# zwizwa/synth_tools

Hardware: NVIDIA B200
Metric: voice-samples/sec (higher is better)
Workload: dtype u32

## Files before the change

### synth_tools_b200/csrc/common.cuh

```cuda
#pragma once
#include <cuda_runtime.h>
#include <stdint.h>
#include <string>
#include <vector>
#include "../../include/cproc_cuda.h"

#define CPROC_N_SM 148

struct cproc_cuda_ctx {
    int device = 0;
    cudaStream_t stream = nullptr;
    cudaStream_t copy_stream = nullptr;
    cudaStream_t aux_stream = nullptr;
    cudaEvent_t aux_ev[17] = {};
    bool own_stream = false;
    cudaEvent_t ev0 = nullptr, ev1 = nullptr;
    std::string err;
    uint64_t launches = 0;
    int pdm_block = 64;
    int pdm_tpb = 2;
    int pdm_stage = 1;
    int pdm_ws = 1;
    int pdm_tlog = 7;
    int pdm_v1_chains = 2;
    int pdm_planar_bulk = 2;
    int pdm_ctas_per_sm = 4;
    int pdm_slice_batches = 64;
    uint32_t *d_work = nullptr;
    uint32_t *d_sm_rank = nullptr;
    uint32_t *d_jump[5] = {nullptr, nullptr, nullptr, nullptr, nullptr};
    uint32_t *d_jump16 = nullptr;
    int pdm_persist = 1;
    int pdm_warps_per_smsp = 1;
    int n_sm = CPROC_N_SM;
    int voice_fpt = 0;
    int grain_block = 128;
    int grain_blocks_per_sm = 2;
    int grain_bulk = 5;
    int grain_vec4 = 1;
    int grain_mix2 = 2;
    int planar_bulk = 2;
    int graph_vec4 = 1;
    int graph_jit = 1;
    int xvoice_vpt = 0;
    int xvoice_mix2_per_sm = 0;
    int xvoice_mix2_blocks = 0;
    int xvoice_mix2 = 1;
    int xvoice_groups = 0;
    int xvoice_chunk = 0;
    uint64_t opt_epoch = 0;
    int run_graph = 2;
    int xvoice_closed = 1;
};

struct cproc_graph_jit {
    int state = 0;
    std::vector<char> cubin;
    cudaLibrary_t lib = nullptr;
    cudaKernel_t k_il = nullptr, k_il4 = nullptr, k_pl = nullptr, k_ps = nullptr, k_pt = nullptr;
    uint32_t pl_smem = 0, pl_block = 0, pt_smem = 0;
};

struct cproc_cuda_bus;
struct cproc_cuda_batch {
    cproc_cuda_ctx *ctx = nullptr;
    cproc_cuda_bus *bus = nullptr; uint32_t bus_mode = 0;
    cproc_cuda_config cfg{};
    std::vector<cproc_cuda_node> nodes;
    std::vector<uint32_t> node_off;
    std::vector<uint32_t> outs;
    uint64_t n = 0;
    uint64_t npad = 0;
    uint64_t n_banks = 0;
    uint64_t n_bus = 0;
    uint32_t state_words = 0, param_words = 0;
    uint32_t *d_state = nullptr;
    uint32_t *d_param = nullptr;
    uint32_t *d_prng = nullptr;
    uint32_t *d_prng2 = nullptr;
    uint32_t *d_prng_g = nullptr;
    cproc_cuda_node *d_nodes = nullptr;
    uint32_t count = 0;
    void *d_in = nullptr, *d_in2 = nullptr, *d_ctl = nullptr, *d_out = nullptr, *d_mix = nullptr;
    size_t cap_in = 0, cap_in2 = 0, cap_ctl = 0, cap_out = 0, cap_mix = 0;
    void *d_out2 = nullptr; size_t cap_out2 = 0;
    uint32_t *d_aux = nullptr; bool aux_dirty = true; uint32_t aux_weird = 0;
    void *d_scratch = nullptr; size_t cap_scratch = 0;
    uint32_t *d_acc = nullptr; size_t cap_acc = 0;
    unsigned long long *d_flags = nullptr;
    uint64_t n_flags = 0;
    unsigned long long epoch = 0;
    cproc_graph_jit jit[2];
    std::vector<uint32_t> ev_in, ev_chg, ev_out;
    std::string jit_log;
    struct run_graph {
        uint64_t F = 0; uint32_t layout = 0; size_t sz[5] = {0, 0, 0, 0, 0};
        uint64_t opt_epoch = 0;
        int seen = 0;
        cudaGraphExec_t exec = nullptr; uint32_t kernels = 0;
        uint8_t *h = nullptr; size_t cap = 0;
    } rg;
    uint32_t *st_h = nullptr; bool ride_state = false;
};

int cproc_set_err(cproc_cuda_ctx *ctx, int code, const char *fmt, ...);
int cproc_check(cproc_cuda_ctx *ctx, cudaError_t e, const char *what);

#define CK(ctx, call) do { int _rc = cproc_check((ctx), (call), #call); if (_rc) return _rc; } while (0)
#define CK_LAUNCH(ctx, name) do { (ctx)->launches++; int _rc = cproc_check((ctx), cudaGetLastError(), name); if (_rc) return _rc; } while (0)

struct cproc_kind_meta {
    const char *name;
    uint32_t n_state; const char *state[5]; uint32_t state_f;
    uint32_t n_param; const char *param[3]; uint32_t param_f;
    uint32_t n_input; const char *input[2]; uint32_t input_f;
    uint32_t n_config; const char *config[1];
};
static const cproc_kind_meta k_cproc_kinds[CPROC_CUDA_NODE_KINDS] = {
    {"acc",      1, {"out"}, 0,                                    0, {nullptr}, 0,                               1, {"in"}, 0,           0, {nullptr}},
    {"edge",     2, {"out", "last"}, 0,                            0, {nullptr}, 0,                               1, {"in"}, 0,           0, {nullptr}},
    {"glide",    5, {"out", "vel0", "pos1", "vel1", "count"}, 0,   0, {nullptr}, 0,                               1, {"in"}, 0,           1, {"div_log"}},
    {"pdm",      5, {"out", "s1", "s2", "s3", "s4"}, 0,            0, {nullptr}, 0,                               2, {"in", "dither"}, 0, 1, {"order_shift"}},
    {"phasor_f", 2, {"out", "phase"}, 1,                           1, {"inc"}, 0,                                 1, {"mod"}, 0,          0, {nullptr}},
    {"svf",      2, {"out", "bp"}, 3,                              2, {"f", "q"}, 3,                              1, {"in"}, 1,           0, {nullptr}},
    {"env",      3, {"out", "env", "t"}, 3,                        3, {"attack", "release", "gate_frames"}, 3,    1, {"in"}, 1,           0, {nullptr}},
    {"onepole",  1, {"out"}, 1,                                    1, {"a"}, 1,                                   1, {"in"}, 1,           0, {nullptr}},
    {"gain",     1, {"out"}, 1,                                    1, {"g"}, 1,                                   1, {"in"}, 1,           0, {nullptr}},
    {"asfloat",  1, {"out"}, 1,                                    0, {nullptr}, 0,                               1, {"in"}, 0,           0, {nullptr}},
    {"glide_f",  3, {"out", "step", "count"}, 3,                   0, {nullptr}, 0,                               1, {"in"}, 1,           1, {"div_log"}},
    {"mul",      1, {"out"}, 1,                                    0, {nullptr}, 0,                               2, {"in", "gain"}, 3,   0, {nullptr}},
};
static inline bool cproc_kind_out_float(uint32_t type) { const uint32_t k = CPROC_CUDA_NODE_KIND(type); return k < CPROC_CUDA_NODE_KINDS && (k_cproc_kinds[k].state_f & 1u); }
static inline uint32_t cproc_node_words(uint32_t type) {
    const uint32_t kind = CPROC_CUDA_NODE_KIND(type);
    if (kind == CPROC_CUDA_NODE_PDM) return 1u + (CPROC_CUDA_NODE_ARG(type) & 7u);
    return kind < CPROC_CUDA_NODE_KINDS ? k_cproc_kinds[kind].n_state : 1u;
}
static inline uint32_t cproc_node_param_words(uint32_t type) {
    const uint32_t kind = CPROC_CUDA_NODE_KIND(type);
    return kind < CPROC_CUDA_NODE_KINDS ? k_cproc_kinds[kind].n_param : 0u;
}
static inline const char *cproc_node_check(const cproc_cuda_node *nodes, uint32_t k, uint32_t n_inputs) {
    const cproc_cuda_node &nd = nodes[k];
    const uint32_t kind = CPROC_CUDA_NODE_KIND(nd.type), arg = CPROC_CUDA_NODE_ARG(nd.type);
    if (kind >= CPROC_CUDA_NODE_KINDS || (nd.type >> 16)) return "unknown node type";
    if ((kind == CPROC_CUDA_NODE_GLIDE || kind == CPROC_CUDA_NODE_GLIDE_F) && (arg < 1 || arg > 24)) return "glide needs a control divider log2 of 1..24";
    if (kind == CPROC_CUDA_NODE_PDM && ((arg & 7u) < 1 || (arg & 7u) > 4)) return "pdm order must be 1..4";
    if (kind != CPROC_CUDA_NODE_GLIDE && kind != CPROC_CUDA_NODE_GLIDE_F && kind != CPROC_CUDA_NODE_PDM && arg) return "this processor takes no config word";
    const cproc_kind_meta &m = k_cproc_kinds[kind];
    for (uint32_t j = 0; j < m.n_input; ++j) {
        const int32_t src = j ? nd.src2 : nd.src;
        if (src == CPROC_CUDA_SRC_ZERO) { if (kind <= CPROC_CUDA_NODE_PDM) return "input not connected"; continue; }
        if (src >= (int32_t)k) return j ? "second input reads a node that is not bound yet (ANF)" : "reads a node that is not bound yet (ANF)";
        if (src < 0 && (uint32_t)(-(src + 1)) >= n_inputs) return j ? "second input reads an input stream that does not exist" : "reads an input stream that does not exist";
        if (src >= 0 && cproc_kind_out_float(nodes[src].type) && !((m.input_f >> j) & 1u)) return "a float output feeds an integer input (undefined in C for negative values)";
    }
    return nullptr;
}
static inline uint64_t ceil_div_u64(uint64_t a, uint64_t b) { return (a + b - 1) / b; }

struct cproc_io_sizes { size_t in, in2, ctl, out, mix; };
int cproc_io_bytes(const cproc_cuda_batch *b, uint64_t F, const cproc_cuda_io *io, cproc_io_sizes *s);

int launch_graph(cproc_cuda_batch *b, uint64_t F, const cproc_cuda_io *io);
int launch_graph_scan(cproc_cuda_batch *b, uint64_t F, const cproc_cuda_io *io);
int cproc_graph_jit_get(cproc_cuda_batch *b, bool has_changed, cproc_graph_jit **out);
int launch_pdm(cproc_cuda_batch *b, uint64_t F, const cproc_cuda_io *io);
int launch_pdm_v1(cproc_cuda_batch *b, uint64_t F, const cproc_cuda_io *io);
int launch_pdm_v2(cproc_cuda_batch *b, uint64_t F, const cproc_cuda_io *io);
int launch_pwm(cproc_cuda_batch *b, uint64_t F, const cproc_cuda_io *io);
int launch_voice_bank(cproc_cuda_batch *b, uint64_t F, const cproc_cuda_io *io);
int launch_square_grain(cproc_cuda_batch *b, uint64_t F, const cproc_cuda_io *io);
int launch_square_grain_mix(cproc_cuda_batch *b, uint64_t F, const cproc_cuda_io *io);
int launch_xvoice(cproc_cuda_batch *b, uint64_t F, const cproc_cuda_io *io);
int launch_onepole(cproc_cuda_batch *b, uint64_t F, const cproc_cuda_io *io);
int launch_word_clock(cproc_cuda_batch *b, uint64_t F, const cproc_cuda_io *io);

__global__ void k_imix_to_float(const int32_t *imix, float *mix, uint64_t count, float scale);
__global__ void k_voice_finish(const int32_t *isum, float *vec, uint64_t count, uint32_t mode);

__device__ __forceinline__ uint32_t xorshift32_step(uint32_t x) {
    x ^= x << 13;
    x ^= x >> 17;
    x ^= x << 5;
    return x;
}

__device__ __forceinline__ void st_v4_stream(void *p, uint4 v) {
    asm volatile("st.global.cs.v4.u32 [%0], {%1, %2, %3, %4};" ::"l"(p), "r"(v.x), "r"(v.y), "r"(v.z), "r"(v.w) : "memory");
}
__device__ __forceinline__ uint4 ld_v4_stream(const void *p) {
    uint4 v;
    asm volatile("ld.global.cs.v4.u32 {%0, %1, %2, %3}, [%4];" : "=r"(v.x), "=r"(v.y), "=r"(v.z), "=r"(v.w) : "l"(p));
    return v;
}
```

### synth_tools_b200/csrc/k_pdm_v2.cu

```cuda
#include "common.cuh"
#include "pdm_common.cuh"
#include "planar_bulk.cuh"

struct PdmV2Params {
    uint32_t *st;
    uint64_t npad, n, n_banks;
    uint32_t bank_size;
    const uint32_t *prng;
    uint32_t *prng_out;
    const uint32_t *dither_ext;
    const uint32_t *setpoints;
    uint8_t *out;
    uint64_t F;
    uint32_t count0, ctl_div_log, sh, dmask, layout;
    uint32_t m1;
};

template <int K, int B>
struct V2Regs {
    uint32_t sp[B], p0[B], v0[B], p1[B], v1[B], s[B][K];
    __device__ __forceinline__ void load(const uint32_t *st, uint64_t npad, uint64_t c0) {
#pragma unroll
        for (int j = 0; j < B; ++j) {
            const uint32_t *x = st + c0 + j;
            sp[j] = __ldcg(x); p0[j] = __ldcg(x + npad); v0[j] = __ldcg(x + 2 * npad);
            p1[j] = __ldcg(x + 3 * npad); v1[j] = __ldcg(x + 4 * npad);
#pragma unroll
            for (int k = 0; k < K; ++k) s[j][k] = __ldcg(x + (5 + k) * npad);
        }
    }
    __device__ __forceinline__ void zero() {
#pragma unroll
        for (int j = 0; j < B; ++j) {
            sp[j] = p0[j] = v0[j] = p1[j] = v1[j] = 0;
#pragma unroll
            for (int k = 0; k < K; ++k) s[j][k] = 0;
        }
    }
    __device__ __forceinline__ void store(uint32_t *st, uint64_t npad, uint64_t c0) const {
#pragma unroll
        for (int j = 0; j < B; ++j) {
            uint32_t *x = st + c0 + j;
            __stcg(x, sp[j]); __stcg(x + npad, p0[j]); __stcg(x + 2 * npad, v0[j]);
            __stcg(x + 3 * npad, p1[j]); __stcg(x + 4 * npad, v1[j]);
#pragma unroll
            for (int k = 0; k < K; ++k) __stcg(x + (5 + k) * npad, s[j][k]);
        }
    }
    __device__ __forceinline__ void boundary(const uint32_t *row, uint64_t c0, uint64_t n, uint32_t L) {
#pragma unroll
        for (int j = 0; j < B; ++j) {
            if (row && c0 + j < n) sp[j] = __ldg(row + c0 + j);
            p0[j] = p1[j]; v0[j] = v1[j];
            p1[j] += v1[j] << L;
            v1[j] = (uint32_t)((int32_t)(sp[j] - p1[j]) >> L);
        }
    }
    template <bool FASTQ, bool DEXT>
    __device__ __forceinline__ void group(uint32_t &rng, const uint32_t *dext16, uint32_t sh, uint32_t dmask, uint32_t m1, uint32_t (&w)[B][4]) {
        uint32_t dbuf[16];
        if (DEXT) {
#pragma unroll
            for (int i = 0; i < 4; ++i) {
                uint4 v = *reinterpret_cast<const uint4 *>(dext16 + i * 4);
                dbuf[4 * i] = v.x; dbuf[4 * i + 1] = v.y; dbuf[4 * i + 2] = v.z; dbuf[4 * i + 3] = v.w;
            }
        }
        uint32_t a[B][4];
#pragma unroll
        for (int i = 0; i < 16; ++i) {
            uint32_t d;
            if (DEXT) d = dbuf[i] & dmask;
            else { rng = xorshift32_step(rng); asm("and.b32 %0, %1, %2;" : "=r"(d) : "r"(rng), "r"(dmask)); }
#pragma unroll
            for (int j = 0; j < B; ++j) {
                p0[j] += v0[j];
                if (FASTQ) a[j][i & 3] = pdm_step_q24<K>(s[j], p0[j], d, m1);
                else a[j][i & 3] = pdm_step<K>(s[j], p0[j], sh, d);
                if ((i & 3) == 3)
                    w[j][i >> 2] = FASTQ ? pack_top_bytes(a[j][0], a[j][1], a[j][2], a[j][3])
                                         : pack_low_bytes(a[j][0], a[j][1], a[j][2], a[j][3]);
            }
        }
    }
};

__device__ __forceinline__ uint64_t v2_rows_before(uint32_t count0, uint32_t div, uint64_t t0) {
    const uint64_t first = count0 == 0 ? 0 : div - count0;
    return t0 > first ? 1 + (t0 - first - 1) / div : 0;
}

template <int K, int B, bool TPB, bool FASTQ, bool DEXT>
__global__ void __launch_bounds__(128) k_pdm_v2_simple(const PdmV2Params p) {
    const uint64_t tid = (uint64_t)blockIdx.x * blockDim.x + threadIdx.x;
    if (tid >= (TPB ? p.n_banks : p.n_banks * p.bank_size)) return;
    const uint64_t c0 = tid * B;
    const uint64_t bank = TPB ? tid : tid / p.bank_size;
    const bool rng_owner = TPB ? true : (tid % p.bank_size == 0);
    V2Regs<K, B> r;
    r.load(p.st, p.npad, c0);
    uint32_t rng = __ldg(p.prng + bank);
    const uint32_t L = p.ctl_div_log, div_mask = (1u << L) - 1u;
    uint32_t cnt = p.count0;
    uint64_t row = 0;
    const uint32_t *dext = DEXT ? p.dither_ext + bank * p.F : nullptr;
    const bool tiled = p.layout == CPROC_CUDA_TILED;
    for (uint64_t g = 0; g < (p.F >> 4); ++g) {
        if (cnt == 0) {
            r.boundary(p.setpoints ? p.setpoints + row * p.n : nullptr, c0, p.n, L);
            ++row;
        }
        uint32_t w[B][4];
        r.template group<FASTQ, DEXT>(rng, DEXT ? dext + (g << 4) : nullptr, p.sh, p.dmask, p.m1, w);
#pragma unroll
        for (int j = 0; j < B; ++j) {
            if (c0 + j < p.n) {
                uint8_t *dst = tiled ? p.out + ((g * p.n + c0 + j) << 4) : p.out + (c0 + j) * p.F + (g << 4);
                st_v4_stream(dst, make_uint4(w[j][0], w[j][1], w[j][2], w[j][3]));
            }
        }
        cnt = (cnt + 16) & div_mask;
    }
    r.store(p.st, p.npad, c0);
    if (rng_owner && !DEXT) p.prng_out[bank] = rng;
}

template <int K>
__global__ void k_pdm_v2_any(const PdmV2Params p) {
    const uint64_t c = (uint64_t)blockIdx.x * blockDim.x + threadIdx.x;
    if (c >= p.n_banks * p.bank_size) return;
    const uint64_t bank = c / p.bank_size;
    uint32_t *x = p.st + c;
    uint32_t sp = x[0], p0 = x[p.npad], v0 = x[2 * p.npad], p1 = x[3 * p.npad], v1 = x[4 * p.npad], s[K];
#pragma unroll
    for (int k = 0; k < K; ++k) s[k] = x[(5 + k) * p.npad];
    uint32_t rng = __ldg(p.prng + bank);
    const uint32_t L = p.ctl_div_log, div_mask = (1u << L) - 1u;
    uint32_t cnt = p.count0;
    uint64_t row = 0;
    const uint32_t *dext = p.dither_ext ? p.dither_ext + bank * p.F : nullptr;
    for (uint64_t t = 0; t < p.F; ++t) {
        uint32_t d = dext ? dext[t] : (rng = xorshift32_step(rng));
        d &= p.dmask;
        if (cnt == 0) {
            if (p.setpoints && c < p.n) sp = p.setpoints[row * p.n + c];
            p0 = p1; v0 = v1;
            p1 += v1 << L;
            v1 = (uint32_t)((int32_t)(sp - p1) >> L);
            ++row;
        }
        p0 += v0;
        uint32_t q = pdm_step<K>(s, p0, p.sh, d);
        if (c < p.n) {
            uint64_t idx = p.layout == CPROC_CUDA_TILED ? (((t >> 4) * p.n + c) << 4) + (t & 15)
                         : p.layout == CPROC_CUDA_INTERLEAVED ? t * p.n + c
                         : c * p.F + t;
            p.out[idx] = (uint8_t)q;
        }
        cnt = (cnt + 1) & div_mask;
    }
    x[0] = sp; x[p.npad] = p0; x[2 * p.npad] = v0; x[3 * p.npad] = p1; x[4 * p.npad] = v1;
#pragma unroll
    for (int k = 0; k < K; ++k) x[(5 + k) * p.npad] = s[k];
    if (!dext && c % p.bank_size == 0) p.prng_out[bank] = rng;
}

#define WS4_BAR_FULL 1
#define WS4_BAR_EMPTY 3
template <int ID, int N> __device__ __forceinline__ void bar_sync_i() { asm volatile("bar.sync %0, %1;" ::"n"(ID), "n"(N) : "memory"); }
template <int ID, int N> __device__ __forceinline__ void bar_arrive_i() { asm volatile("bar.arrive %0, %1;" ::"n"(ID), "n"(N) : "memory"); }
template <int BASE, int N> __device__ __forceinline__ void bar_sync_slot(uint32_t s) { if (s) bar_sync_i<BASE + 1, N>(); else bar_sync_i<BASE, N>(); }
template <int BASE, int N> __device__ __forceinline__ void bar_arrive_slot(uint32_t s) { if (s) bar_arrive_i<BASE + 1, N>(); else bar_arrive_i<BASE, N>(); }

struct PdmV2Work {
    uint32_t *counter;
    unsigned long long *flags;
    unsigned long long epoch;
    uint32_t groups, slices, bps;
    uint32_t *prng_g;
    uint32_t *sm_rank;
    const uint32_t *jump;
};

template <int K>
__device__ __forceinline__ uint32_t ws4_tick(uint32_t &p0, uint32_t v0, uint32_t (&s)[K], uint32_t d, uint32_t m1) {
    p0 += v0;
    if constexpr (K == 2) {
        const uint32_t x = s[0] + p0;
        const uint32_t a = lop3_and_or(s[1], d);
        s[0] = imad(a, m1, x);
        s[1] = s[1] + s[0] - a;
        return a;
    } else {
        return pdm_step_q24<K>(s, p0, d, m1);
    }
}

template <int NT, int TLOG>
__device__ __noinline__ uint32_t ws4_producer_arith(uint4 *dbuf, const uint32_t (*jt)[256], uint32_t x0, uint32_t dmask, uint64_t batches, uint32_t lane) {
    constexpr int QW = (1 << TLOG) / 4, QC = QW / 2;
    uint32_t xa = x0, s = 0;
    for (uint64_t bt = 0; bt < batches; ++bt) {
        uint32_t xb = jump_apply(jt, xa);
        if (bt >= 2) bar_sync_slot<WS4_BAR_EMPTY, NT>(s);
        uint4 *slot = dbuf + s * (QW * 32) + lane;
#pragma unroll 4
        for (int q = 0; q < QC; ++q) {
            uint4 va, vb;
            xa = xorshift32_step(xa); va.x = xa & dmask;
            xb = xorshift32_step(xb); vb.x = xb & dmask;
            xa = xorshift32_step(xa); va.y = xa & dmask;
            xb = xorshift32_step(xb); vb.y = xb & dmask;
            xa = xorshift32_step(xa); va.z = xa & dmask;
            xb = xorshift32_step(xb); vb.z = xb & dmask;
            xa = xorshift32_step(xa); va.w = xa & dmask;
            xb = xorshift32_step(xb); vb.w = xb & dmask;
            slot[q * 32] = va;
            slot[(QC + q) * 32] = vb;
        }
        xa = xb;
        __threadfence_block();
        bar_arrive_slot<WS4_BAR_FULL, NT>(s);
        s ^= 1u;
    }
    return xa;
}

constexpr size_t ws4_smem_bytes(int CW, int TLOG, int PL) {
    return (size_t)(PL == 2 ? CW * 2 * 4096 : PL == 1 ? CW * 4096 : 0) + 2 * ((1u << TLOG) / 4) * 32 * 16 + 4096 + 1024;
}

template <int K, int CW, int TLOG, int PL>
__global__ void __launch_bounds__(32 * (CW + 1)) k_pdm_v2_ws4(const PdmV2Params p, const PdmV2Work wk, const __grid_constant__ CUtensorMap tm_out) {
    constexpr int T = 1 << TLOG, NT = 32 * (CW + 1);
    constexpr int QW = T / 4;
    extern __shared__ __align__(1024) uint8_t ws4_smem[];
    uint8_t *base = ws4_smem + ((1024u - ((uint32_t)__cvta_generic_to_shared(ws4_smem) & 1023u)) & 1023u);
    uint8_t *pbox = base;
    uint4 *dbuf = reinterpret_cast<uint4 *>(base + (PL == 2 ? CW * 2 * 4096 : PL == 1 ? CW * 4096 : 0));
    uint32_t *tab = reinterpret_cast<uint32_t *>(dbuf + 2 * QW * 32);
    for (uint32_t i = threadIdx.x; i < 1024; i += NT) tab[i] = __ldg(wk.jump + i);
    __shared__ uint32_t rank_s, smsp_s[CW + 1], item_s;
    const uint32_t warp = threadIdx.x >> 5, lane = threadIdx.x & 31;
    if (threadIdx.x == 0) {
        uint32_t smid;
        asm volatile("mov.u32 %0, %%smid;" : "=r"(smid));
        rank_s = atomicAdd(wk.sm_rank + smid, 1u);
    }
    if (lane == 0) {
        uint32_t wid;
        asm volatile("mov.u32 %0, %%warpid;" : "=r"(wid));
        smsp_s[warp] = wid & 3u;
    }
    __syncthreads();
    uint32_t prod_warp = 0;
#pragma unroll
    for (int w = CW; w >= 0; --w) if (smsp_s[w] == (rank_s & 3u)) prod_warp = w;
    const uint32_t cw = warp - (warp > prod_warp ? 1u : 0u);
    const uint32_t cl = cw * 32 + lane;
    const uint32_t L = p.ctl_div_log, period = 1u << (L - TLOG);
    const uint32_t m1 = p.m1, bs = p.bank_size;
    const uint64_t batches_total = p.F >> TLOG;
    const uint64_t n_ch = p.n_banks * bs;
    const uint32_t total = wk.groups * wk.slices;
    for (;;) {
        if (threadIdx.x == 0) {
            const uint32_t idx = atomicAdd(wk.counter, 1u);
            item_s = idx;
            if (idx < total) {
                const uint32_t g = idx % wk.groups, sl = idx / wk.groups;
                const unsigned long long want = (wk.epoch << 32) | sl;
                if (sl) while (ld_acquire_u64(wk.flags + g) != want) __nanosleep(64);
            }
        }
        __syncthreads();
        const uint32_t idx = item_s;
        if (idx >= total) break;
        const uint32_t g = idx % wk.groups, sl = idx / wk.groups;
        const uint64_t bt0 = (uint64_t)sl * wk.bps;
        const uint64_t nb = batches_total - bt0 < wk.bps ? batches_total - bt0 : wk.bps;
        const uint64_t c_lo = (uint64_t)g * (32 * CW);
        const uint64_t bank_lo = c_lo / bs;
        if (warp == prod_warp) {
            const uint64_t bank = bank_lo + lane;
            const bool have = bank < p.n_banks;
            uint32_t x = 1u;
            if (have) x = sl ? __ldcg(wk.prng_g + (uint64_t)g * 32 + lane) : __ldg(p.prng + bank);
            x = ws4_producer_arith<NT, TLOG>(dbuf, reinterpret_cast<const uint32_t (*)[256]>(tab), x, p.dmask, nb, lane);
            if (have) {
                if (sl + 1 < wk.slices) __stcg(wk.prng_g + (uint64_t)g * 32 + lane, x);
                else if (bank * bs >= c_lo && bank * bs < c_lo + 32 * CW) p.prng_out[bank] = x;
            }
        } else {
            const uint64_t c = c_lo + cl;
            const bool live = c < n_ch;
            const uint32_t bl = live ? (uint32_t)(c / bs - bank_lo) : 0u;
            V2Regs<K, 1> r;
            if (live) r.load(p.st, p.npad, c); else r.zero();
            const uint32_t cb = (uint32_t)(((p.count0 >> TLOG) + bt0) & (period - 1));
            uint32_t until = cb == 0 ? 0 : period - cb;
            const uint32_t *sp_row = p.setpoints ? p.setpoints + v2_rows_before(p.count0, 1u << L, bt0 << TLOG) * p.n : nullptr;
            const bool store = c < p.n;
            uint8_t *dst = p.layout == CPROC_CUDA_TILED ? p.out + (((bt0 << (TLOG - 4)) * p.n + c) << 4) : p.out + c * p.F + (bt0 << TLOG);
            const uint64_t dstep = p.layout == CPROC_CUDA_TILED ? p.n << 4 : 16;
            const uint32_t pbox_s = PL == 2 ? (uint32_t)__cvta_generic_to_shared(pbox + cw * 8192) : PL == 1 ? (uint32_t)__cvta_generic_to_shared(pbox) : 0u;
            const uint4 *dlane = dbuf + bl;
            uint32_t s = 0;
            for (uint64_t bt = 0; bt < nb; ++bt) {
                if (until == 0) {
                    r.boundary(sp_row, c, p.n, L);
                    if (sp_row) sp_row += p.n;
                    until = period;
                }
                --until;
                bar_sync_slot<WS4_BAR_FULL, NT>(s);
                const uint4 *dslot = dlane + s * (QW * 32);
#pragma unroll
                for (int g16 = 0; g16 < T / 16; ++g16) {
                    uint32_t w[4];
#pragma unroll
                    for (int i4 = 0; i4 < 4; ++i4) {
                        const uint4 dv = dslot[(g16 * 4 + i4) * 32];
                        const uint32_t d[4] = {dv.x, dv.y, dv.z, dv.w};
                        uint32_t a[4];
#pragma unroll
                        for (int i = 0; i < 4; ++i) a[i] = ws4_tick<K>(r.p0[0], r.v0[0], r.s[0], d[i], m1);
                        if constexpr (PL == 1) {
                            const uint32_t row = (((uint32_t)bt << TLOG) + g16 * 16 + i4 * 4) & 127u;
#pragma unroll
                            for (int i = 0; i < 4; ++i)
                                asm volatile("st.shared.u8 [%0], %1;" ::"r"(pbox_s + (row + i) * (32u * CW) + cl), "r"(a[i] >> 24) : "memory");
                        } else w[i4] = pack_top_bytes(a[0], a[1], a[2], a[3]);
                    }
                    if constexpr (PL == 1) {
                        const uint32_t tk = ((uint32_t)bt << TLOG) + g16 * 16;
                        if ((tk & 127u) == 112u) {
                            bar_sync_i<5, 32 * CW>();
                            const uint64_t tick0 = (bt0 << TLOG) + tk - 112;
#pragma unroll
                            for (int i = 0; i < 8; ++i) {
                                const uint32_t piece = i * (32u * CW) + cl, row = piece / (2u * CW), col = piece % (2u * CW);
                                if (c_lo + col * 16 < p.n) {
                                    uint4 v;
                                    asm volatile("ld.shared.v4.u32 {%0, %1, %2, %3}, [%4];" : "=r"(v.x), "=r"(v.y), "=r"(v.z), "=r"(v.w) : "r"(pbox_s + piece * 16u));
                                    st_v4_stream(p.out + (tick0 + row) * p.n + c_lo + col * 16, v);
                                }
                            }
                        }
                    } else if constexpr (PL == 2) {
                        const uint32_t tk = ((uint32_t)bt << TLOG) + g16 * 16;
                        const uint32_t box = (tk >> 7) & 1u, ch = (tk >> 4) & 7u;
                        if (ch == 0 && tk >= 256) {
                            if (lane == 0) asm volatile("cp.async.bulk.wait_group.read 1;" ::: "memory");
                            __syncwarp();
                        }
                        asm volatile("st.shared.v4.u32 [%0], {%1, %2, %3, %4};" ::"r"(pbox_s + box * 4096u + lane * 128u + ((ch ^ (lane & 7u)) << 4)),
                                     "r"(w[0]), "r"(w[1]), "r"(w[2]), "r"(w[3]) : "memory");
                        if (ch == 7) {
                            asm volatile("fence.proxy.async.shared::cta;" ::: "memory");
                            __syncwarp();
                            if (lane == 0) {
                                asm volatile("cp.async.bulk.tensor.2d.global.shared::cta.tile.bulk_group [%0, {%1, %2}], [%3];"
                                             ::"l"(reinterpret_cast<uint64_t>(&tm_out)), "r"((int32_t)((bt0 << TLOG) + tk - 112)), "r"((int32_t)(c_lo + cw * 32)),
                                               "r"(pbox_s + box * 4096u) : "memory");
                                asm volatile("cp.async.bulk.commit_group;" ::: "memory");
                            }
                        }
                    } else {
                        if (store) st_v4_stream(dst, make_uint4(w[0], w[1], w[2], w[3]));
                        dst += dstep;
                    }
                }
                if (bt + 2 < nb) bar_arrive_slot<WS4_BAR_EMPTY, NT>(s);
                s ^= 1u;
            }
            if constexpr (PL == 2) {
                if (lane == 0) asm volatile("cp.async.bulk.wait_group.read 0;" ::: "memory");
                __syncwarp();
            }
            if (live) r.store(p.st, p.npad, c);
        }
        __syncthreads();
        if (threadIdx.x == 0) {
            __threadfence();
            st_release_u64(wk.flags + g, (wk.epoch << 32) | (sl + 1));
        }
    }
    if (threadIdx.x == 0) {
        const uint32_t left = atomicAdd(wk.counter + 1, 1u);
        if (left == gridDim.x - 1) { wk.counter[0] = 0; wk.counter[1] = 0; __threadfence(); }
    }
}


static int ws4_jump(cproc_cuda_ctx *ctx, int tlog, const uint32_t **out) {
    uint32_t *&d = ctx->d_jump[tlog - 6];
    if (!d) {
        std::vector<uint32_t> h(1024);
        jump_table_fill(h.data(), 1u << (tlog - 1));
        CK(ctx, cudaMalloc(&d, h.size() * 4));
        CK(ctx, cudaMemcpyAsync(d, h.data(), h.size() * 4, cudaMemcpyHostToDevice, ctx->stream));
        CK(ctx, cudaStreamSynchronize(ctx->stream));
    }
    *out = d;
    return 0;
}

template <int K, int CW, int TLOG, int PL>
static int ws4_go(cproc_cuda_ctx *ctx, const PdmV2Params &p, PdmV2Work &wk, const CUtensorMap &tm, uint64_t slice_ticks) {
    auto kern = k_pdm_v2_ws4<K, CW, TLOG, PL>;
    constexpr size_t smem = ws4_smem_bytes(CW, TLOG, PL);
    static int occ = 0;
    if (!occ) {
        CK(ctx, cudaFuncSetAttribute(kern, cudaFuncAttributeMaxDynamicSharedMemorySize, (int)smem));
        CK(ctx, cudaOccupancyMaxActiveBlocksPerMultiprocessor(&occ, kern, 32 * (CW + 1), smem));
        if (occ < 1) { occ = 0; return cproc_set_err(ctx, CPROC_CUDA_ECUDA, "pdm_v2: kernel does not fit an SM (%zu bytes of shared memory)", smem); }
    }
    const uint64_t batches = p.F >> TLOG;
    uint64_t bps = slice_ticks >> TLOG;
    if (PL != 0 && TLOG < 7) bps &= ~(uint64_t)((128 >> TLOG) - 1);
    if (bps < 1) bps = PL != 0 && TLOG < 7 ? (128 >> TLOG) : 1;
    wk.bps = (uint32_t)bps;
    wk.slices = (uint32_t)ceil_div_u64(batches, bps);
    if ((uint64_t)wk.groups * wk.slices >= 0xFFFFFFFFull) return cproc_set_err(ctx, CPROC_CUDA_EINVAL, "pdm_v2: too many work items; render fewer ticks per call");
    int want_per_sm = ctx->pdm_ctas_per_sm;
    if (CW == 1 && want_per_sm < 6) want_per_sm = 6;
    const int per_sm = want_per_sm < occ ? want_per_sm : occ;
    uint64_t grid = (uint64_t)ctx->n_sm * per_sm;
    if (grid > wk.groups) grid = wk.groups;
    kern<<<(unsigned)grid, 32 * (CW + 1), smem, ctx->stream>>>(p, wk, tm);
    return 0;
}

template <int K, int CW>
static int ws4_dispatch(cproc_cuda_ctx *ctx, const PdmV2Params &p, PdmV2Work &wk, const CUtensorMap &tm, int tlog, int pl, uint64_t slice_ticks) {
    if (pl == 1) return ws4_go<K, CW, 7, 1>(ctx, p, wk, tm, slice_ticks);
    if (pl == 2) return ws4_go<K, CW, 6, 2>(ctx, p, wk, tm, slice_ticks);
    if (tlog >= 7) return ws4_go<K, CW, 7, 0>(ctx, p, wk, tm, slice_ticks);
    return ws4_go<K, CW, 6, 0>(ctx, p, wk, tm, slice_ticks);
}

template <int K>
static int launch_v2_ws4(cproc_cuda_batch *b, PdmV2Params &p) {
    cproc_cuda_ctx *ctx = b->ctx;
    const int CW = p.bank_size <= 4 ? (int)p.bank_size : 4;
    CUtensorMap tm;
    memset(&tm, 0, sizeof(tm));
    int pl = 0;
    if (p.layout == CPROC_CUDA_PLANAR && ctx->pdm_planar_bulk && (p.F % 128) == 0 && pbulk::encode_rows_u8(&tm, p.out, p.F, p.n)) pl = 2;
    if (p.layout == CPROC_CUDA_INTERLEAVED) pl = 1;
    int tlog = pl == 2 ? 6 : pl == 1 ? 7 : ctx->pdm_tlog;
    if (tlog > 6 && (((p.F | p.count0) & 127u) || p.ctl_div_log < 7)) tlog = 6;
    PdmV2Work wk;
    memset(&wk, 0, sizeof(wk));
    wk.groups = (uint32_t)ceil_div_u64(p.n_banks * p.bank_size, 32 * CW);
    if (b->n_flags < wk.groups) {
        if (b->d_flags) cudaFree(b->d_flags);
        if (b->d_prng_g) cudaFree(b->d_prng_g);
        b->d_flags = nullptr; b->d_prng_g = nullptr; b->n_flags = 0;
        CK(ctx, cudaMalloc(&b->d_flags, sizeof(unsigned long long) * wk.groups));
        CK(ctx, cudaMemsetAsync(b->d_flags, 0, sizeof(unsigned long long) * wk.groups, ctx->stream));
        CK(ctx, cudaMalloc(&b->d_prng_g, sizeof(uint32_t) * 32 * wk.groups));
        b->n_flags = wk.groups;
    }
    if (!ctx->d_work) {
        CK(ctx, cudaMalloc(&ctx->d_work, 2 * sizeof(uint32_t)));
        CK(ctx, cudaMemsetAsync(ctx->d_work, 0, 2 * sizeof(uint32_t), ctx->stream));
    }
    if (!ctx->d_sm_rank) {
        CK(ctx, cudaMalloc(&ctx->d_sm_rank, 1024 * sizeof(uint32_t)));
        CK(ctx, cudaMemsetAsync(ctx->d_sm_rank, 0, 1024 * sizeof(uint32_t), ctx->stream));
    }
    wk.counter = ctx->d_work; wk.flags = b->d_flags; wk.epoch = ++b->epoch; wk.prng_g = b->d_prng_g; wk.sm_rank = ctx->d_sm_rank;
    int rc;
    if ((rc = ws4_jump(ctx, tlog, &wk.jump))) return rc;
    const uint64_t slice_ticks = (uint64_t)ctx->pdm_slice_batches * 64;
    switch (CW) {
    case 1: return ws4_dispatch<K, 1>(ctx, p, wk, tm, tlog, pl, slice_ticks);
    case 2: return ws4_dispatch<K, 2>(ctx, p, wk, tm, tlog, pl, slice_ticks);
    case 3: return ws4_dispatch<K, 3>(ctx, p, wk, tm, tlog, pl, slice_ticks);
    default: return ws4_dispatch<K, 4>(ctx, p, wk, tm, tlog, pl, slice_ticks);
    }
}

template <int K, bool FASTQ>
static int launch_v2_order(cproc_cuda_batch *b, PdmV2Params &p, bool fast, bool dext) {
    cproc_cuda_ctx *ctx = b->ctx;
    if (!fast) {
        k_pdm_v2_any<K><<<(unsigned)ceil_div_u64(p.npad, 128), 128, 0, ctx->stream>>>(p);
        return 0;
    }
    if constexpr (FASTQ) {
        if (!dext && ctx->pdm_ws && (p.F % 64) == 0 && (p.count0 % 64) == 0 && p.ctl_div_log >= 6) return launch_v2_ws4<K>(b, p);
    }
    const int blk = ctx->pdm_block;
    const bool tpb = ctx->pdm_tpb && p.bank_size <= 4;
#define V2_SIMPLE(BB, TT) do { \
        const unsigned grid = (unsigned)ceil_div_u64((TT) ? p.n_banks : p.n_banks * p.bank_size, blk); \
        if (dext) k_pdm_v2_simple<K, BB, TT, FASTQ, true><<<grid, blk, 0, ctx->stream>>>(p); \
        else k_pdm_v2_simple<K, BB, TT, FASTQ, false><<<grid, blk, 0, ctx->stream>>>(p); } while (0)
    if (tpb) {
        switch (p.bank_size) {
        case 1: V2_SIMPLE(1, true); break;
        case 2: V2_SIMPLE(2, true); break;
        case 3: V2_SIMPLE(3, true); break;
        default: V2_SIMPLE(4, true); break;
        }
    } else V2_SIMPLE(1, false);
#undef V2_SIMPLE
    return 0;
}

int launch_pdm_v2(cproc_cuda_batch *b, uint64_t F, const cproc_cuda_io *io) {
    cproc_cuda_ctx *ctx = b->ctx;
    const cproc_cuda_config &c = b->cfg;
    if (!io->out) return cproc_set_err(ctx, CPROC_CUDA_EINVAL, "pdm_v2: out is NULL");
    if (io->layout == CPROC_CUDA_TILED && (F & 15)) return cproc_set_err(ctx, CPROC_CUDA_EINVAL, "pdm_v2: TILED needs F %% 16 == 0");
    if (F == 0) return 0;
    uint32_t div = 1u << c.ctl_div_log;
    if (io->ctl) {
        const uint64_t first = b->count == 0 ? 0 : div - b->count;
        const uint64_t rows = F > first ? 1 + (F - first - 1) / div : 0;
        if (rows > io->n_ctl) return cproc_set_err(ctx, CPROC_CUDA_EINVAL, "pdm_v2: run crosses %llu control boundaries but ctl has %u rows", (unsigned long long)rows, io->n_ctl);
    }
    if (!b->d_prng2) CK(ctx, cudaMalloc(&b->d_prng2, sizeof(uint32_t) * b->n_banks));
    PdmV2Params p;
    p.st = b->d_state; p.npad = b->npad; p.n = b->n; p.n_banks = b->n_banks; p.bank_size = c.bank_size;
    p.prng = b->d_prng; p.prng_out = b->d_prng2; p.dither_ext = (const uint32_t *)io->in2; p.setpoints = (const uint32_t *)io->ctl;
    p.out = (uint8_t *)io->out; p.F = F; p.count0 = b->count; p.ctl_div_log = c.ctl_div_log; p.sh = c.out_shift;
    p.dmask = c.dither_mask; p.layout = io->layout; p.m1 = 0xFFFFFFFFu;
    const bool aligned_ptr = ((uintptr_t)io->out & 15) == 0 && (!io->in2 || ((uintptr_t)io->in2 & 15) == 0);
    const bool fastq = c.out_shift == 24 && (c.dither_mask & 0xFF000000u) == 0;
    const bool dext = io->in2 != nullptr;
    const bool il_fast = io->layout == CPROC_CUDA_INTERLEAVED && fastq && !dext && ctx->pdm_ws && ((F | b->count) & 127) == 0 && c.ctl_div_log >= 7 && (b->n & 15) == 0;
    const bool fast = (F & 15) == 0 && (b->count & 15) == 0 && c.ctl_div_log >= 4 && aligned_ptr &&
                      (io->layout == CPROC_CUDA_TILED || io->layout == CPROC_CUDA_PLANAR || il_fast);
    int rc;
#define V2_ORDER(KK) (fastq ? launch_v2_order<KK, true>(b, p, fast, dext) : launch_v2_order<KK, false>(b, p, fast, dext))
    switch (c.order) {
    case 1: rc = V2_ORDER(1); break;
    case 2: rc = V2_ORDER(2); break;
    case 3: rc = V2_ORDER(3); break;
    default: rc = V2_ORDER(4); break;
    }
#undef V2_ORDER
    if (rc) return rc;
    CK_LAUNCH(ctx, "k_pdm_v2");
    if (!dext) { uint32_t *t = b->d_prng; b->d_prng = b->d_prng2; b->d_prng2 = t; }
    b->count = (uint32_t)((b->count + F) & (div - 1));
    return 0;
}
```

Baseline: 2986 billion.

## Pipeline work items across producer and consumers in warp-specialized PDM kernel

The producer warp now claims work items on its own and passes each item index to the consumer warps through the full/empty double-buffer barriers. This removes the block-wide __syncthreads between items, so the producer can start generating dither for the next item while consumers finish the current one. The dependency flag release moves to a consumer-only named barrier, and the producer publishes the PRNG state early so the next slice can start sooner. The change also moves the occupancy cache into a per-context map and calls cudaFuncSetAttribute on every launch, which adds a small host cost and makes the barrier protocol more complex and more prone to deadlock.

```diff
diff --git a/synth_tools_b200/csrc/common.cuh b/synth_tools_b200/csrc/common.cuh
--- a/synth_tools_b200/csrc/common.cuh
+++ b/synth_tools_b200/csrc/common.cuh
@@ -1,6 +1,7 @@
 #pragma once
 #include <cuda_runtime.h>
 #include <stdint.h>
+#include <map>
 #include <string>
 #include <vector>
 #include "../../include/cproc_cuda.h"
@@ -26,6 +27,7 @@
     int pdm_planar_bulk = 2;
     int pdm_ctas_per_sm = 4;
     int pdm_slice_batches = 64;
+    std::map<const void *, int> pdm_ws4_occ;
     uint32_t *d_work = nullptr;
     uint32_t *d_sm_rank = nullptr;
     uint32_t *d_jump[5] = {nullptr, nullptr, nullptr, nullptr, nullptr};
diff --git a/synth_tools_b200/csrc/k_pdm_v2.cu b/synth_tools_b200/csrc/k_pdm_v2.cu
--- a/synth_tools_b200/csrc/k_pdm_v2.cu
+++ b/synth_tools_b200/csrc/k_pdm_v2.cu
@@ -197,12 +197,14 @@
 }
 
 template <int NT, int TLOG>
-__device__ __noinline__ uint32_t ws4_producer_arith(uint4 *dbuf, const uint32_t (*jt)[256], uint32_t x0, uint32_t dmask, uint64_t batches, uint32_t lane) {
+__device__ __noinline__ uint32_t ws4_producer_arith(uint4 *dbuf, const uint32_t (*jt)[256], uint32_t x0, uint32_t dmask, uint64_t batches,
+                                                    uint64_t seq, uint32_t lane, uint32_t *desc, uint32_t item, uint32_t *x_out) {
     constexpr int QW = (1 << TLOG) / 4, QC = QW / 2;
-    uint32_t xa = x0, s = 0;
+    uint32_t xa = x0, s = (uint32_t)seq & 1u;
     for (uint64_t bt = 0; bt < batches; ++bt) {
         uint32_t xb = jump_apply(jt, xa);
-        if (bt >= 2) bar_sync_slot<WS4_BAR_EMPTY, NT>(s);
+        if (seq + bt >= 2) bar_sync_slot<WS4_BAR_EMPTY, NT>(s);
+        if (bt == 0 && lane == 0) *desc = item;
         uint4 *slot = dbuf + s * (QW * 32) + lane;
 #pragma unroll 4
         for (int q = 0; q < QC; ++q) {
@@ -219,6 +221,7 @@
             slot[(QC + q) * 32] = vb;
         }
         xa = xb;
+        if (x_out && bt + 1 == batches) { __stcg(x_out, xa); __threadfence(); }
         __threadfence_block();
         bar_arrive_slot<WS4_BAR_FULL, NT>(s);
         s ^= 1u;
@@ -240,7 +243,7 @@
     uint4 *dbuf = reinterpret_cast<uint4 *>(base + (PL == 2 ? CW * 2 * 4096 : PL == 1 ? CW * 4096 : 0));
     uint32_t *tab = reinterpret_cast<uint32_t *>(dbuf + 2 * QW * 32);
     for (uint32_t i = threadIdx.x; i < 1024; i += NT) tab[i] = __ldg(wk.jump + i);
-    __shared__ uint32_t rank_s, smsp_s[CW + 1], item_s;
+    __shared__ uint32_t rank_s, smsp_s[CW + 1], item_s[2];
     const uint32_t warp = threadIdx.x >> 5, lane = threadIdx.x & 31;
     if (threadIdx.x == 0) {
         uint32_t smid;
@@ -263,35 +266,53 @@
     const uint64_t batches_total = p.F >> TLOG;
     const uint64_t n_ch = p.n_banks * bs;
     const uint32_t total = wk.groups * wk.slices;
-    for (;;) {
-        if (threadIdx.x == 0) {
-            const uint32_t idx = atomicAdd(wk.counter, 1u);
-            item_s = idx;
-            if (idx < total) {
-                const uint32_t g = idx % wk.groups, sl = idx / wk.groups;
-                const unsigned long long want = (wk.epoch << 32) | sl;
-                if (sl) while (ld_acquire_u64(wk.flags + g) != want) __nanosleep(64);
-            }
-        }
-        __syncthreads();
-        const uint32_t idx = item_s;
-        if (idx >= total) break;
-        const uint32_t g = idx % wk.groups, sl = idx / wk.groups;
-        const uint64_t bt0 = (uint64_t)sl * wk.bps;
-        const uint64_t nb = batches_total - bt0 < wk.bps ? batches_total - bt0 : wk.bps;
-        const uint64_t c_lo = (uint64_t)g * (32 * CW);
-        const uint64_t bank_lo = c_lo / bs;
-        if (warp == prod_warp) {
-            const uint64_t bank = bank_lo + lane;
+    if (warp == prod_warp) {
+        uint64_t seq = 0;
+        for (uint32_t par = 0;; par ^= 1u) {
+            uint32_t idx = 0;
+            if (lane == 0) {
+                idx = atomicAdd(wk.counter, 1u);
+                if (idx < total) {
+                    const uint32_t g = idx % wk.groups, sl = idx / wk.groups;
+                    const unsigned long long want = (wk.epoch << 32) | sl;
+                    if (sl) while (ld_acquire_u64(wk.flags + g) != want) __nanosleep(64);
+                }
+            }
+            idx = __shfl_sync(0xFFFFFFFFu, idx, 0);
+            __syncwarp();
+            if (idx >= total) {
+                if (seq >= 2) bar_sync_slot<WS4_BAR_EMPTY, NT>((uint32_t)seq & 1u);
+                if (lane == 0) item_s[par] = idx;
+                __threadfence_block();
+                bar_arrive_slot<WS4_BAR_FULL, NT>((uint32_t)seq & 1u);
+                if (seq >= 1) bar_sync_slot<WS4_BAR_EMPTY, NT>((uint32_t)(seq - 1) & 1u);
+                break;
+            }
+            const uint32_t g = idx % wk.groups, sl = idx / wk.groups;
+            const uint64_t bt0 = (uint64_t)sl * wk.bps;
+            const uint64_t nb = batches_total - bt0 < wk.bps ? batches_total - bt0 : wk.bps;
+            const uint64_t c_lo = (uint64_t)g * (32 * CW);
+            const uint64_t bank = c_lo / bs + lane;
             const bool have = bank < p.n_banks;
             uint32_t x = 1u;
             if (have) x = sl ? __ldcg(wk.prng_g + (uint64_t)g * 32 + lane) : __ldg(p.prng + bank);
-            x = ws4_producer_arith<NT, TLOG>(dbuf, reinterpret_cast<const uint32_t (*)[256]>(tab), x, p.dmask, nb, lane);
-            if (have) {
-                if (sl + 1 < wk.slices) __stcg(wk.prng_g + (uint64_t)g * 32 + lane, x);
-                else if (bank * bs >= c_lo && bank * bs < c_lo + 32 * CW) p.prng_out[bank] = x;
-            }
-        } else {
+            uint32_t *x_out = have && sl + 1 < wk.slices ? wk.prng_g + (uint64_t)g * 32 + lane : nullptr;
+            x = ws4_producer_arith<NT, TLOG>(dbuf, reinterpret_cast<const uint32_t (*)[256]>(tab), x, p.dmask, nb, seq, lane, item_s + par, idx, x_out);
+            if (have && sl + 1 == wk.slices && bank * bs >= c_lo && bank * bs < c_lo + 32 * CW) p.prng_out[bank] = x;
+            seq += nb;
+        }
+    } else {
+        const uint32_t pbox_s = PL == 2 ? (uint32_t)__cvta_generic_to_shared(pbox + cw * 8192) : PL == 1 ? (uint32_t)__cvta_generic_to_shared(pbox) : 0u;
+        uint32_t s = 0;
+        for (uint32_t par = 0;; par ^= 1u) {
+            bar_sync_slot<WS4_BAR_FULL, NT>(s);
+            const uint32_t idx = item_s[par];
+            if (idx >= total) break;
+            const uint32_t g = idx % wk.groups, sl = idx / wk.groups;
+            const uint64_t bt0 = (uint64_t)sl * wk.bps;
+            const uint64_t nb = batches_total - bt0 < wk.bps ? batches_total - bt0 : wk.bps;
+            const uint64_t c_lo = (uint64_t)g * (32 * CW);
+            const uint64_t bank_lo = c_lo / bs;
             const uint64_t c = c_lo + cl;
             const bool live = c < n_ch;
             const uint32_t bl = live ? (uint32_t)(c / bs - bank_lo) : 0u;
@@ -303,9 +324,7 @@
             const bool store = c < p.n;
             uint8_t *dst = p.layout == CPROC_CUDA_TILED ? p.out + (((bt0 << (TLOG - 4)) * p.n + c) << 4) : p.out + c * p.F + (bt0 << TLOG);
             const uint64_t dstep = p.layout == CPROC_CUDA_TILED ? p.n << 4 : 16;
-            const uint32_t pbox_s = PL == 2 ? (uint32_t)__cvta_generic_to_shared(pbox + cw * 8192) : PL == 1 ? (uint32_t)__cvta_generic_to_shared(pbox) : 0u;
             const uint4 *dlane = dbuf + bl;
-            uint32_t s = 0;
             for (uint64_t bt = 0; bt < nb; ++bt) {
                 if (until == 0) {
                     r.boundary(sp_row, c, p.n, L);
@@ -313,7 +332,7 @@
                     until = period;
                 }
                 --until;
-                bar_sync_slot<WS4_BAR_FULL, NT>(s);
+                if (bt) bar_sync_slot<WS4_BAR_FULL, NT>(s);
                 const uint4 *dslot = dlane + s * (QW * 32);
 #pragma unroll
                 for (int g16 = 0; g16 < T / 16; ++g16) {
@@ -371,7 +390,7 @@
                         dst += dstep;
                     }
                 }
-                if (bt + 2 < nb) bar_arrive_slot<WS4_BAR_EMPTY, NT>(s);
+                bar_arrive_slot<WS4_BAR_EMPTY, NT>(s);
                 s ^= 1u;
             }
             if constexpr (PL == 2) {
@@ -379,13 +398,16 @@
                 __syncwarp();
             }
             if (live) r.store(p.st, p.npad, c);
-        }
-        __syncthreads();
-        if (threadIdx.x == 0) {
-            __threadfence();
-            st_release_u64(wk.flags + g, (wk.epoch << 32) | (sl + 1));
-        }
-    }
+            if (sl + 1 < wk.slices) {
+                bar_sync_i<6, 32 * CW>();
+                if (cl == 0) {
+                    __threadfence();
+                    st_release_u64(wk.flags + g, (wk.epoch << 32) | (sl + 1));
+                }
+            }
+        }
+    }
+    __syncthreads();
     if (threadIdx.x == 0) {
         const uint32_t left = atomicAdd(wk.counter + 1, 1u);
         if (left == gridDim.x - 1) { wk.counter[0] = 0; wk.counter[1] = 0; __threadfence(); }
@@ -410,9 +432,9 @@
 static int ws4_go(cproc_cuda_ctx *ctx, const PdmV2Params &p, PdmV2Work &wk, const CUtensorMap &tm, uint64_t slice_ticks) {
     auto kern = k_pdm_v2_ws4<K, CW, TLOG, PL>;
     constexpr size_t smem = ws4_smem_bytes(CW, TLOG, PL);
-    static int occ = 0;
+    CK(ctx, cudaFuncSetAttribute(kern, cudaFuncAttributeMaxDynamicSharedMemorySize, (int)smem));
+    int &occ = ctx->pdm_ws4_occ[(const void *)kern];
     if (!occ) {
-        CK(ctx, cudaFuncSetAttribute(kern, cudaFuncAttributeMaxDynamicSharedMemorySize, (int)smem));
         CK(ctx, cudaOccupancyMaxActiveBlocksPerMultiprocessor(&occ, kern, 32 * (CW + 1), smem));
         if (occ < 1) { occ = 0; return cproc_set_err(ctx, CPROC_CUDA_ECUDA, "pdm_v2: kernel does not fit an SM (%zu bytes of shared memory)", smem); }
     }
```

Result: no change. 3011 billion (median of 6 runs) (+0.9%).
